# gnychis/gnuradio-3.5.0-dmr

Measured on AMD Instinct MI355X. Metric: Msamples/s through FIR->demod chain @256 taps, higher is better.
Workload: dtype f32 (FIR operands split into two binary16 halves on the matrix cores, f32 accumulation; demodulator f32)

## Files before the change

### gnuradio-3.5.0-dmr_amd/csrc/fir_mfma.hip

```cpp
#include <cstdio>
#include <cstdlib>

#include "device_math.h"
#include "fir_kernels.h"
#include "grhip_internal.h"
#include "mfma_tables.h"

#ifndef GRHIP_LG_W2
#define GRHIP_LG_W2 0
#endif
#ifndef GRHIP_LG_ACC3
#define GRHIP_LG_ACC3 0
#endif
#ifndef GRHIP_LG_ORDER
#define GRHIP_LG_ORDER 1
#endif
#ifndef GRHIP_MF_WGS
#define GRHIP_MF_WGS 2
#endif
#ifndef GRHIP_LG_SPF
#define GRHIP_LG_SPF 0
#endif
#ifndef GRHIP_LG_MAX4
#define GRHIP_LG_MAX4 0
#endif
#ifndef GRHIP_LG_EPI2
#define GRHIP_LG_EPI2 0
#endif
#ifndef GRHIP_LG_STAGE2
#define GRHIP_LG_STAGE2 1
#endif
#ifndef GRHIP_LG_LEAN
#define GRHIP_LG_LEAN 0
#endif
#ifndef GRHIP_LG_SPREAD
#define GRHIP_LG_SPREAD 0
#endif


namespace grhip {

typedef _Float16 h16x8 __attribute__((ext_vector_type(8)));
typedef _Float16 h16x2 __attribute__((ext_vector_type(2)));
typedef float f32x4 __attribute__((ext_vector_type(4)));
typedef float f32x2 __attribute__((ext_vector_type(2)));
typedef unsigned int u32x4 __attribute__((ext_vector_type(4)));
typedef unsigned int u32x2 __attribute__((ext_vector_type(2)));
typedef const float __attribute__((address_space(4))) *cfloat_cp;

namespace {

__host__ __device__ constexpr int ilog2c(int v) { return v <= 1 ? 0 : 1 + ilog2c(v >> 1); }

constexpr int SCR_SEG = 36;
constexpr int SCR_WAVE = mf::SEGS * SCR_SEG;

template <int D, int KS> struct Geo {
    static constexpr int Q = mf::SEG_OUT * D;
    static constexpr int LOGQ = ilog2c(Q);
    static constexpr int CB = mf::BLK * D / mf::CHUNK;
    static constexpr int NCH = mf::chunks_per_seg(D, KS);
    static constexpr int SP = mf::tile_samples(D, KS);
    static constexpr int NI = mf::rounds(D, KS);
    static constexpr int PL = mf::plane_bytes(D, KS);
    static constexpr int HALO = NCH * mf::CHUNK - (mf::SEGS * mf::SEG_OUT - mf::WAVE_NEW) * D - (mf::SEGS - 1) * 0;
    static constexpr int OFF_ATAN = 4 * PL;
    static constexpr int OFF_MISC = OFF_ATAN + 256 * 8;
    static constexpr int OFF_G = OFF_MISC + 32;
    static constexpr int LDS = OFF_G + mf::NG * 64 * 16;
    static_assert((1 << LOGQ) == Q, "segment stride must be a power of two");
    static_assert(HALO >= 0 && HALO % 32 == 0, "halo");
    static_assert(mf::NBLK != 4 || mf::plane_pos(mf::WAVE_NEW * D - 1, D) + 2 - mf::plane_pos(HALO, D) >= SCR_WAVE * 4, "a wave's own stretch of a plane must hold one accumulator tile");
    static_assert(mf::ROUND % Q == 0, "a staging round must cover whole segment strides");
};

#define GRHIP_DPPF(v, ctrl, rmask, bc) \
    __builtin_bit_cast(float, __builtin_amdgcn_update_dpp(0, __builtin_bit_cast(int, (v)), (ctrl), (rmask), 0xf, (bc)))
__device__ __forceinline__ float wave_max_nonneg(float x)
{
    x = __builtin_fmaxf(x, GRHIP_DPPF(x, 0xB1, 0xf, true));
    x = __builtin_fmaxf(x, GRHIP_DPPF(x, 0x4E, 0xf, true));
    x = __builtin_fmaxf(x, GRHIP_DPPF(x, 0x141, 0xf, true));
    x = __builtin_fmaxf(x, GRHIP_DPPF(x, 0x140, 0xf, true));
    x = __builtin_fmaxf(x, GRHIP_DPPF(x, 0x142, 0xa, false));
    x = __builtin_fmaxf(x, GRHIP_DPPF(x, 0x143, 0xc, false));
    return __builtin_bit_cast(float, __builtin_amdgcn_readlane(__builtin_bit_cast(int, x), 63));
}

__device__ __forceinline__ float wave_sum_f(float x)
{
    x += GRHIP_DPPF(x, 0xB1, 0xf, true);
    x += GRHIP_DPPF(x, 0x4E, 0xf, true);
    x += GRHIP_DPPF(x, 0x141, 0xf, true);
    x += GRHIP_DPPF(x, 0x140, 0xf, true);
    x += GRHIP_DPPF(x, 0x142, 0xa, false);
    x += GRHIP_DPPF(x, 0x143, 0xc, false);
    return __builtin_bit_cast(float, __builtin_amdgcn_readlane(__builtin_bit_cast(int, x), 63));
}

template <int CTRL>
__device__ __forceinline__ float dpp_row(float v)
{
    return __builtin_bit_cast(float, __builtin_amdgcn_update_dpp(0, __builtin_bit_cast(int, v), CTRL, 0xf, 0xf, true));
}

__device__ __forceinline__ h16x2 split_lo(f32x2 x, h16x2 hi)
{
    unsigned lo;
    const unsigned h = __builtin_bit_cast(unsigned, hi);
    asm("v_fma_mixlo_f16 %0, %1, 1.0, -%2 op_sel_hi:[0,0,1]" : "=v"(lo) : "v"(x.x), "v"(h));
    asm("v_fma_mixhi_f16 %0, %1, 1.0, -%2 op_sel:[0,0,1] op_sel_hi:[0,0,1]" : "+v"(lo) : "v"(x.y), "v"(h));
    return __builtin_bit_cast(h16x2, lo);
}

__device__ __forceinline__ void split_scaled(float x0, float x1, float s, h16x2 &hi, h16x2 &lo)
{
    unsigned h, l;
    asm("v_fma_mixlo_f16 %0, %1, %2, 0" : "=v"(h) : "v"(x0), "v"(s));
    asm("v_fma_mixhi_f16 %0, %1, %2, 0" : "+v"(h) : "v"(x1), "v"(s));
    asm("v_fma_mixlo_f16 %0, %1, %2, -%3 op_sel_hi:[0,0,1]" : "=v"(l) : "v"(x0), "v"(s), "v"(h));
    asm("v_fma_mixhi_f16 %0, %1, %2, -%3 op_sel:[0,0,1] op_sel_hi:[0,0,1]" : "+v"(l) : "v"(x1), "v"(s), "v"(h));
    hi = __builtin_bit_cast(h16x2, h);
    lo = __builtin_bit_cast(h16x2, l);
}

#ifdef GRHIP_STAMP
__device__ unsigned long long *g_mf_stamp_buf = nullptr;
__device__ __forceinline__ unsigned long long mf_stamp_now()
{
    unsigned long long t;
    __builtin_amdgcn_sched_barrier(0);
    asm volatile("s_memrealtime %0\n\ts_waitcnt lgkmcnt(0)" : "=s"(t) :: "memory");
    __builtin_amdgcn_sched_barrier(0);
    return t;
}
#define MF_STAMP_DECL unsigned long long st_acc[8] = {0, 0, 0, 0, 0, 0, 0, 0}, st_last = mf_stamp_now(), st_begin = st_last
#define MF_STAMP(k) do { unsigned long long n__ = mf_stamp_now(); st_acc[k] += n__ - st_last; st_last = n__; } while (0)
#define MF_STAMP_OUT(nwaves) do { if ((threadIdx.x & 63) == 0 && g_mf_stamp_buf) { \
        unsigned long long *o__ = g_mf_stamp_buf + ((size_t)blockIdx.x * (nwaves) + (threadIdx.x >> 6)) * 10; \
        for (int k__ = 0; k__ < 8; ++k__) o__[k__] = st_acc[k__]; \
        o__[8] = st_begin; o__[9] = mf_stamp_now(); } } while (0)
#else
#define MF_STAMP_DECL
#define MF_STAMP(k)
#define MF_STAMP_OUT(nwaves)
#endif

struct AtanPairs {
    const f32x2 *p;
    __device__ __forceinline__ f32x2 operator[](int k) const { return p[k]; }
};

}

template <int D, int KS, bool PREMIX, int EPI, bool TAPQ = false>
__global__ void __launch_bounds__(mf::THREADS, GRHIP_MF_WGS) fir_mfma_kernel(const FirMfmaArgs a)
{
    static_assert(!TAPQ || PREMIX, "the tap-angle correction belongs to freq_xlating's pre-mix form");
    using G = Geo<D, KS>;
    constexpr int NI = G::NI, PL = G::PL, LOGQ = G::LOGQ, CB = G::CB, SP = G::SP;
    constexpr bool DEMOD = EPI == EPI_DEMOD;
    constexpr bool ROT = EPI == EPI_ROTATE;
    static_assert(!DEMOD || PREMIX, "the fused demodulator belongs to the pre-mix form");
    static_assert(EPI == EPI_DEMOD || EPI == EPI_ROTATE || EPI == EPI_NONE, "epilogue");
    constexpr int NTE = mf::NTE, BLK = mf::BLK, NBLK = mf::NBLK;

    extern __shared__ __attribute__((aligned(256))) unsigned char smem[];
    const AtanPairs s_atan{reinterpret_cast<const f32x2 *>(smem + G::OFF_ATAN)};
    float *wmax = reinterpret_cast<float *>(smem + G::OFF_MISC);
    unsigned *sched_slot = reinterpret_cast<unsigned *>(smem + G::OFF_MISC + 16);

    const int t = threadIdx.x, lane = t & 63, w = t >> 6;
    const int tiles_per_stream = (int)((a.n_out + NTE - 1) / NTE);

    h16x8 Ah[KS], Al[KS];
    {
        const h16x8 *Ag = reinterpret_cast<const h16x8 *>(a.A);
#pragma unroll
        for (int js = 0; js < KS; ++js) {
            Ah[js] = Ag[(js * 2 + 0) * 64 + lane];
            Al[js] = Ag[(js * 2 + 1) * 64 + lane];
        }
    }
    constexpr int JG0 = mf::g_first(KS);
    if (TAPQ) {
        const h16x8 *Gg = reinterpret_cast<const h16x8 *>(a.A) + (size_t)KS * 2 * 64;
        if (t < mf::NG * 64) reinterpret_cast<h16x8 *>(smem + G::OFF_G)[t] = Gg[t];
    }
    const float tq_sgn = __builtin_amdgcn_ldexpf((lane & 8) ? 1.0f : -1.0f, -mf::G_EXTRA_EXP);
    f32x2 wl{1.f, 0.f}, wl1{1.f, 0.f};
    if (PREMIX) {
        const float2 v = a.wlane[t];
        wl = f32x2{v.x, v.y};
        wl1 = cmul_pk(wl, f32x2{a.wstep.x, a.wstep.y});
    }
    const cfloat_cp stab = (cfloat_cp)a.stab;
    if (DEMOD) {
        f32x2 *at = reinterpret_cast<f32x2 *>(smem + G::OFF_ATAN);
        for (int i = t; i < 256; i += mf::THREADS)
            at[i] = GRHIP_LG_LEAN ? f32x2{a.atan_tab[i], a.atan_tab[i + 1] - a.atan_tab[i]} : f32x2{a.atan_tab[i], a.atan_tab[i + 1]};
    }
    const int st_off = 4 * t + 32 * ((2 * t) >> LOGQ);
    constexpr int ST_STEP = 2 * mf::ROUND + 32 * (mf::ROUND >> LOGQ);
    const int col = lane & 15, part = col >> 3, sl = col & 7, g = lane >> 4;
    const int rd_u = w * (mf::WAVE_NEW * D) + (sl << LOGQ) + 8 * g;
    const int rd_plane = part * 2 * PL;
    const int scw_u = w * (mf::WAVE_NEW * D) + G::HALO;
    float *scw = reinterpret_cast<float *>(smem + 2 * scw_u + 32 * (scw_u >> LOGQ));
    const int sc_wr = sl * SCR_SEG + 8 * g + part;
    const int rsl = lane >> 3, r8 = lane & 7;
    const int sc_rd = rsl * SCR_SEG + 4 * r8;

    f32x4 pf[NI];

    const int lead = a.off ^ (int)(a.n_lo & 1);
    auto tile_geom = [&](int s, int b, __amdgpu_buffer_rsrc_t &rsrc, int &voff) __attribute__((always_inline)) {
        const long long g0 = ((long long)b * NTE - BLK) * D - a.off - a.n_lo + lead;
        const float2 *x = a.x + (long long)s * a.x_stride + a.n_lo - lead;
        const long long bytes = (a.n_in - a.n_lo + lead) * 8;
        rsrc = __builtin_amdgcn_make_buffer_rsrc(const_cast<float2 *>(x), 0, (int)bytes, 0x00020000);
        voff = (int)(g0 * 8) + 16 * t;
    };
    auto fetch = [&](__amdgpu_buffer_rsrc_t rsrc, int voff, int part_) __attribute__((always_inline)) {
        constexpr int PER = (NI + NBLK - 1) / NBLK;
#pragma unroll
        for (int i = 0; i < NI; ++i) {
            if (part_ >= 0 && i / PER != part_) continue;
            int vo = voff + i * (16 * mf::THREADS);
            if ((i + 1) * mf::ROUND > SP && 2 * t + i * mf::ROUND >= SP) vo = 0x7ffff000;
            const u32x4 v = __builtin_amdgcn_raw_buffer_load_b128(rsrc, vo, 0, 0);
            pf[i] = __builtin_bit_cast(f32x4, v);
        }
    };

    [[maybe_unused]] auto fetch_one = [&](__amdgpu_buffer_rsrc_t rsrc, int voff, int i) __attribute__((always_inline)) {
        int vo = voff + i * (16 * mf::THREADS);
        if ((i + 1) * mf::ROUND > SP && 2 * t + i * mf::ROUND >= SP) vo = 0x7ffff000;
        const u32x4 v = __builtin_amdgcn_raw_buffer_load_b128(rsrc, vo, 0, 0);
        pf[i] = __builtin_bit_cast(f32x4, v);
    };
    const unsigned total_tiles = (unsigned)tiles_per_stream * (unsigned)a.n_streams;
    const unsigned Gd = gridDim.x;
    unsigned cur = blockIdx.x, nxt = cur + Gd;
    auto decode = [&](unsigned id, int &s_, int &b_) __attribute__((always_inline)) {
        b_ = (int)(id / (unsigned)a.n_streams);
        s_ = (int)(id - (unsigned)b_ * (unsigned)a.n_streams);
    };
    int s = 0, bidx = 0;
    decode(cur, s, bidx);
    if (cur < total_tiles) {
        __amdgpu_buffer_rsrc_t rsrc; int voff;
        tile_geom(s, bidx, rsrc, voff);
        fetch(rsrc, voff, -1);
    }
    unsigned nn_q = 0;
    int voff_cur = 0;
    if (lead) {
        __amdgpu_buffer_rsrc_t rsrc;
        tile_geom(s, bidx, rsrc, voff_cur);
    }

    MF_STAMP_DECL;
    while (cur < total_tiles) {
        int s_nxt, b_nxt;
        MF_STAMP(7);

#if GRHIP_LG_STAGE2
        f32x2 Sa_first{0.f, 0.f}, Sb_first{0.f, 0.f};
        if (PREMIX && GRHIP_LG_SPF) { Sa_first = f32x2{stab[0], stab[1]}; Sb_first = f32x2{stab[2], stab[3]}; }
#endif
        {
            float m = 0.f, m1 = 0.f, m2 = 0.f, m3 = 0.f;
#pragma unroll
            for (int i = 0; i < NI; ++i) {
                if (GRHIP_LG_MAX4 && (i & 1)) {
                    asm("v_max3_f32 %0, |%1|, |%2|, %0" : "+v"(m2) : "v"(pf[i][0]), "v"(pf[i][1]));
                    asm("v_max3_f32 %0, |%1|, |%2|, %0" : "+v"(m3) : "v"(pf[i][2]), "v"(pf[i][3]));
                } else {
                    asm("v_max3_f32 %0, |%1|, |%2|, %0" : "+v"(m) : "v"(pf[i][0]), "v"(pf[i][1]));
                    asm("v_max3_f32 %0, |%1|, |%2|, %0" : "+v"(GRHIP_LG_MAX4 ? m1 : m) : "v"(pf[i][2]), "v"(pf[i][3]));
                }
            }
            if (GRHIP_LG_MAX4) {
                asm("v_max3_f32 %0, %1, %2, %0" : "+v"(m) : "v"(m1), "v"(m2));
                asm("v_max3_f32 %0, %1, %1, %0" : "+v"(m) : "v"(m3));
            }
            m = wave_max_nonneg(m);
            if (!(m < __builtin_inff())) {
                float mf = 0.f;
#pragma unroll
                for (int i = 0; i < NI; ++i)
#pragma unroll
                    for (int e = 0; e < 4; ++e) {
                        const float av = __builtin_fabsf(pf[i][e]);
                        mf = av < __builtin_inff() ? __builtin_fmaxf(mf, av) : mf;
                    }
                m = wave_max_nonneg(mf);
            }
            if (lane == 0) wmax[w] = m;
            if (a.sched && t == 0) sched_slot[0] = nn_q + 2u * Gd;
        }
        MF_STAMP(0);
        __syncthreads();
        MF_STAMP(1);
        if (a.sched && cur != blockIdx.x) nxt = sched_slot[0];
        nxt = (unsigned)__builtin_amdgcn_readfirstlane((int)nxt);
        decode(nxt, s_nxt, b_nxt);
        float scale, inv_scale;
        {
            const float mt = __builtin_fmaxf(__builtin_fmaxf(wmax[0], wmax[1]), __builtin_fmaxf(wmax[2], wmax[3]));
            int k = 14 - __builtin_amdgcn_frexp_expf(mt);
            k = k > 100 ? 100 : (k < -100 ? -100 : k);
            scale = __builtin_amdgcn_ldexpf(1.0f, k);
            inv_scale = __builtin_amdgcn_ldexpf(1.0f, -k - a.kexp);
        }

        if (lead && bidx == 0) {
#pragma unroll
            for (int i = 0; i < NI; ++i)
                if (voff_cur + i * (16 * mf::THREADS) == 0) { pf[i][0] = 0.f; pf[i][1] = 0.f; }
        }
#if defined(GRHIP_DIAG) && defined(GRHIP_MF_EXP)
        const bool exp_off = a.n_out < 0;
#define MF_EXP_SKIP(bit) if (!((GRHIP_MF_EXP & (bit)) && !exp_off))
#else
#define MF_EXP_SKIP(bit)
#endif
#if GRHIP_LG_STAGE2
        if (PREMIX) MF_EXP_SKIP(2)
        {
            const f32x2 ws0 = wl * scale, ws1 = wl1 * scale;
            unsigned char *dst = smem + st_off;
            auto store_round = [&](int i, unsigned rh, unsigned rlo, unsigned ih, unsigned ilo) __attribute__((always_inline)) {
                if ((i + 1) * mf::ROUND <= SP || 2 * t + i * mf::ROUND < SP) {
                    unsigned char *d = dst + i * ST_STEP;
                    *reinterpret_cast<unsigned *>(d) = rh;
                    *reinterpret_cast<unsigned *>(d + PL) = rlo;
                    *reinterpret_cast<unsigned *>(d + 2 * PL) = ih;
                    *reinterpret_cast<unsigned *>(d + 3 * PL) = ilo;
                }
            };
#define MF_CM1(t, a, b) "v_pk_mul_f32 " t ", " a ", " b " op_sel:[1,1] op_sel_hi:[1,0] neg_lo:[0,1]\n\t"
#define MF_CM2(r, a, b, t) "v_pk_fma_f32 " r ", " a ", " b ", " t " op_sel_hi:[0,1,1]\n\t"
            int i = 0;
            f32x2 Sa = Sa_first, Sb = Sb_first;
            if (!GRHIP_LG_SPF) { Sa = f32x2{stab[0], stab[1]}; Sb = f32x2{stab[2], stab[3]}; }
#pragma unroll
            for (; i + 1 < NI; i += 2) {
                f32x2 Sa_n = Sa, Sb_n = Sb;
                if (GRHIP_LG_SPF) {
                    if (i + 2 < NI) Sa_n = f32x2{stab[2 * i + 4], stab[2 * i + 5]};
                    if (i + 3 < NI) Sb_n = f32x2{stab[2 * i + 6], stab[2 * i + 7]};
                } else if (i > 0) {
                    Sa = f32x2{stab[2 * i], stab[2 * i + 1]}; Sb = f32x2{stab[2 * i + 2], stab[2 * i + 3]};
                }
                f32x2 a0{pf[i][0], pf[i][1]}, a1{pf[i][2], pf[i][3]}, b0{pf[i + 1][0], pf[i + 1][1]}, b1{pf[i + 1][2], pf[i + 1][3]};
                f32x2 t0, t1, t2, t3, p0, p1, p2, p3;
                unsigned arh, aih, arl, ail, brh, bih, brl, bil;
                asm(MF_CM1("%0", "%12", "%14") MF_CM1("%1", "%13", "%14") MF_CM1("%2", "%12", "%15") MF_CM1("%3", "%13", "%15")
                    MF_CM2("%4", "%12", "%14", "%0") MF_CM2("%5", "%13", "%14", "%1") MF_CM2("%6", "%12", "%15", "%2") MF_CM2("%7", "%13", "%15", "%3")
                    MF_CM1("%0", "%8", "%4") MF_CM1("%1", "%9", "%5") MF_CM1("%2", "%10", "%6") MF_CM1("%3", "%11", "%7")
                    MF_CM2("%8", "%8", "%4", "%0") MF_CM2("%9", "%9", "%5", "%1") MF_CM2("%10", "%10", "%6", "%2") "v_pk_fma_f32 %11, %11, %7, %3 op_sel_hi:[0,1,1]"
                    : "=&v"(t0), "=&v"(t1), "=&v"(t2), "=&v"(t3), "=&v"(p0), "=&v"(p1), "=&v"(p2), "=&v"(p3),
                      "+v"(a0), "+v"(a1), "+v"(b0), "+v"(b1)
                    : "v"(ws0), "v"(ws1), "s"(Sa), "s"(Sb));
                asm("v_cvt_pk_f16_f32 %0, %8, %10\n\t"
                    "v_cvt_pk_f16_f32 %1, %9, %11\n\t"
                    "v_cvt_pk_f16_f32 %4, %12, %14\n\t"
                    "v_cvt_pk_f16_f32 %5, %13, %15\n\t"
                    "v_fma_mixlo_f16 %2, %8, 1.0, -%0 op_sel_hi:[0,0,1]\n\t"
                    "v_fma_mixlo_f16 %3, %9, 1.0, -%1 op_sel_hi:[0,0,1]\n\t"
                    "v_fma_mixlo_f16 %6, %12, 1.0, -%4 op_sel_hi:[0,0,1]\n\t"
                    "v_fma_mixlo_f16 %7, %13, 1.0, -%5 op_sel_hi:[0,0,1]\n\t"
                    "v_fma_mixhi_f16 %2, %10, 1.0, -%0 op_sel:[0,0,1] op_sel_hi:[0,0,1]\n\t"
                    "v_fma_mixhi_f16 %3, %11, 1.0, -%1 op_sel:[0,0,1] op_sel_hi:[0,0,1]\n\t"
                    "v_fma_mixhi_f16 %6, %14, 1.0, -%4 op_sel:[0,0,1] op_sel_hi:[0,0,1]\n\t"
                    "v_fma_mixhi_f16 %7, %15, 1.0, -%5 op_sel:[0,0,1] op_sel_hi:[0,0,1]"
                    : "=&v"(arh), "=&v"(aih), "=&v"(arl), "=&v"(ail), "=&v"(brh), "=&v"(bih), "=&v"(brl), "=&v"(bil)
                    : "v"(a0.x), "v"(a0.y), "v"(a1.x), "v"(a1.y), "v"(b0.x), "v"(b0.y), "v"(b1.x), "v"(b1.y));
                store_round(i, arh, arl, aih, ail);
                store_round(i + 1, brh, brl, bih, bil);
                if (GRHIP_LG_SPF) { Sa = Sa_n; Sb = Sb_n; }
            }
            if (i < NI) {
                const f32x2 S = GRHIP_LG_SPF ? Sa : f32x2{stab[2 * i], stab[2 * i + 1]};
                f32x2 e0{pf[i][0], pf[i][1]}, e1{pf[i][2], pf[i][3]};
                e0 = cmul_pk(e0, cmul_pk(ws0, S));
                e1 = cmul_pk(e1, cmul_pk(ws1, S));
                const f32x2 re{e0.x, e1.x}, im{e0.y, e1.y};
                const h16x2 rh = __builtin_convertvector(re, h16x2), ih = __builtin_convertvector(im, h16x2);
                const h16x2 rlo = split_lo(re, rh), ilo = split_lo(im, ih);
                store_round(i, __builtin_bit_cast(unsigned, rh), __builtin_bit_cast(unsigned, rlo), __builtin_bit_cast(unsigned, ih),
                            __builtin_bit_cast(unsigned, ilo));
            }
#undef MF_CM1
#undef MF_CM2
        }
        else
#endif
        MF_EXP_SKIP(2)
        {
            const f32x2 ws0 = wl * scale, ws1 = wl1 * scale;
            unsigned char *dst = smem + st_off;
#pragma unroll
            for (int i = 0; i < NI; ++i) {
                f32x2 e0{pf[i][0], pf[i][1]}, e1{pf[i][2], pf[i][3]};
                if (PREMIX) {
#if defined(GRHIP_DIAG) && defined(GRHIP_PROBE) && (GRHIP_PROBE & 2)
                    const double ang0 = a.omega * (double)(2 * t + mf::ROUND * i - a.off);
                    const f32x2 p0{(float)cos(ang0) * scale, (float)sin(ang0) * scale};
                    const f32x2 p1{(float)cos(ang0 + a.omega) * scale, (float)sin(ang0 + a.omega) * scale};
                    e0 = cmul_pk(e0, p0);
                    e1 = cmul_pk(e1, p1);
#else
                    const f32x2 S{stab[2 * i], stab[2 * i + 1]};
                    e0 = cmul_pk(e0, cmul_pk(ws0, S));
                    e1 = cmul_pk(e1, cmul_pk(ws1, S));
#endif
                } else {
                    e0 = e0 * scale;
                    e1 = e1 * scale;
                }
                const f32x2 re{e0.x, e1.x}, im{e0.y, e1.y};
                const h16x2 rh = __builtin_convertvector(re, h16x2), ih = __builtin_convertvector(im, h16x2);
                const h16x2 rlo = split_lo(re, rh), ilo = split_lo(im, ih);
                if ((i + 1) * mf::ROUND <= SP || 2 * t + i * mf::ROUND < SP) {
#if GRHIP_LG_W2
                    const int ad = st_off + i * ST_STEP;
                    asm volatile("ds_write2st64_b32 %0, %1, %2 offset0:0 offset1:%5\n\t"
                                 "ds_write2st64_b32 %0, %3, %4 offset0:%6 offset1:%7"
                                 :: "v"(ad), "v"(rh), "v"(rlo), "v"(ih), "v"(ilo),
                                    "n"(PL / 256), "n"(2 * (PL / 256)), "n"(3 * (PL / 256)) : "memory");
#else
                    unsigned char *d = dst + i * ST_STEP;
                    *reinterpret_cast<h16x2 *>(d) = rh;
                    *reinterpret_cast<h16x2 *>(d + PL) = rlo;
                    *reinterpret_cast<h16x2 *>(d + 2 * PL) = ih;
                    *reinterpret_cast<h16x2 *>(d + 3 * PL) = ilo;
#endif
                }
            }
        }
        float2 ypf = make_float2(0.f, 0.f);
        if (DEMOD && bidx == 0 && a.y_prev) {
            const float2 yp = a.y_prev[s];
            const float2 vm = a.vtab[BLK - 1];
            const float2 q = cmul_fma(yp, make_float2(vm.x, -vm.y));
            const float sc2 = __builtin_amdgcn_ldexpf(scale, a.kexp);
            ypf = make_float2(q.x * sc2, q.y * sc2);
        }
        MF_STAMP(2);
        __syncthreads();
        MF_STAMP(3);

        __amdgpu_buffer_rsrc_t rsrc_n; int voff_n;
        tile_geom(s_nxt, b_nxt, rsrc_n, voff_n);
        if (nxt >= total_tiles) voff_n = 0x7ffff000 - NI * 16 * mf::THREADS;
        if (a.sched && t == 0) nn_q = atomicAdd(a.sched, 1u);

        constexpr int OOB = 0x7ffffff0;
        __amdgpu_buffer_rsrc_t orsrc, grsrc;
        if (DEMOD) {
            orsrc = __builtin_amdgcn_make_buffer_rsrc(a.d_out + (long long)s * a.d_stride, 0, (int)(a.n_out * 4), 0x00020000);
        } else {
            orsrc = __builtin_amdgcn_make_buffer_rsrc(a.y_out + (long long)s * a.y_stride, 0, (int)(a.n_out * 8), 0x00020000);
            if (ROT) grsrc = __builtin_amdgcn_make_buffer_rsrc(const_cast<float2 *>(a.gtab), 0, (int)(a.n_out * 8), 0x00020000);
        }
        const int jt = w * mf::WAVE_NEW + rsl * mf::SEG_OUT + 2 * r8;
        const int n_base = bidx * NTE - BLK + jt;
        const bool first_of_stream = bidx == 0 && t == 7;
        float ypendx = 0.f, ypendy = 0.f;
        float d1_pend = 0.f;
        float y1x = 0.f, y1y = 0.f;
        const float ypfx = ypf.x, ypfy = ypf.y;

        auto epilogue = [&](int b, const f32x4 &v) __attribute__((always_inline)) {
            const float y0x = v[0], y0y = v[1];
            const float y1px = y1x, y1py = y1y;
            y1x = v[2]; y1y = v[3];
            const float2 y0 = make_float2(y0x, y0y);
            const int n = n_base + BLK * b;
            const bool own = !(b == 0 && rsl == 0) && n >= 0;
            if (DEMOD) {
                if (b == 0) {
                    y1x = first_of_stream ? ypfx : y1x;
                    y1y = first_of_stream ? ypfy : y1y;
                }
                float px = dpp_row<0x111>(y1x), py = dpp_row<0x111>(y1y);
                if (b > 0) {
                    const float cx = dpp_row<0x107>(y1px), cy = dpp_row<0x107>(y1py);
                    px = r8 == 0 ? cx : px;
                    py = r8 == 0 ? cy : py;
                } else {
                    ypendx = y0x; ypendy = y0y;
                }
                const float2 prev = make_float2(px, py), y1 = make_float2(y1x, y1y);
                const float d0 = GRHIP_LG_LEAN ? quad_demod_lean(y0, prev, a.gain, s_atan) : quad_demod_fast(y0, prev, a.gain, s_atan);
                const float d1 = GRHIP_LG_LEAN ? quad_demod_lean(y1, y0, a.gain, s_atan) : quad_demod_fast(y1, y0, a.gain, s_atan);
                if (b == 0) d1_pend = d1;
                const bool st_ok = own && !(b == 0 && r8 == 0);
                const f32x2 dd{d0, d1};
                __builtin_amdgcn_raw_buffer_store_b64(__builtin_bit_cast(u32x2, dd), orsrc, st_ok ? 4 * n : OOB, 0, 0);
            } else {
                float2 o0 = y0, o1 = make_float2(y1x, y1y);
                if (PREMIX) {
                    const float4 vv = *reinterpret_cast<const float4 *>(a.vtab + jt + BLK * b);
                    o0 = cmul_fma(o0, make_float2(vv.x, vv.y));
                    o1 = cmul_fma(o1, make_float2(vv.z, vv.w));
                }
                o0.x *= inv_scale; o0.y *= inv_scale; o1.x *= inv_scale; o1.y *= inv_scale;
                if (ROT) {
                    const u32x4 gv = __builtin_amdgcn_raw_buffer_load_b128(grsrc, own ? 8 * n : OOB, 0, 0);
                    const f32x4 gq = __builtin_bit_cast(f32x4, gv);
                    o0 = cmul_ref(o0, make_float2(gq[0], gq[1]));
                    o1 = cmul_ref(o1, make_float2(gq[2], gq[3]));
                }
                const f32x2 oa{o0.x, o0.y}, ob{o1.x, o1.y};
                const int so = own ? 8 * n : OOB;
                __builtin_amdgcn_raw_buffer_store_b64(__builtin_bit_cast(u32x2, oa), orsrc, so, 0, 0);
                __builtin_amdgcn_raw_buffer_store_b64(__builtin_bit_cast(u32x2, ob), orsrc, so + 8, 0, 0);
            }
        };

        auto chunk_ptr = [&](int c) __attribute__((always_inline)) {
            const int u = rd_u + mf::CHUNK * c;
            return smem + rd_plane + 2 * u + 32 * (u >> LOGQ);
        };
        f32x4 acc[NBLK];
#if defined(GRHIP_DIAG) && defined(GRHIP_MF_EXP) && (GRHIP_MF_EXP & 1)
#pragma unroll
        for (int b = 0; b < NBLK; ++b) acc[b] = f32x4{0.f, 0.f, 0.f, 0.f};
#pragma unroll
        for (int q = 0; q < 4; ++q) fetch(rsrc_n, voff_n, q);
        if (exp_off)
#endif
        {
        h16x8 Bh_n = *reinterpret_cast<const h16x8 *>(chunk_ptr(0));
        h16x8 Bl_n = *reinterpret_cast<const h16x8 *>(chunk_ptr(0) + PL);
#pragma unroll
        for (int b = 0; b < NBLK; ++b) {
#if GRHIP_LG_ACC3
            f32x4 m0{0.f, 0.f, 0.f, 0.f}, m1{0.f, 0.f, 0.f, 0.f}, lo{0.f, 0.f, 0.f, 0.f};
#else
            acc[b] = f32x4{0.f, 0.f, 0.f, 0.f};
#endif
            f32x4 tq{0.f, 0.f, 0.f, 0.f};
            auto kstep = [](int q) constexpr { return GRHIP_LG_ORDER ? ((q & 1) ? KS - 1 - (q >> 1) : (q >> 1)) : q; };
            h16x8 Gcur{}, Gnext{};
#pragma unroll
            for (int jq = 0; jq < KS; ++jq) {
                const int j = kstep(jq);
                const h16x8 Bh = Bh_n, Bl = Bl_n;
                if (TAPQ) {
                    Gcur = Gnext;
                    const int jn = jq + 1 < KS ? kstep(jq + 1) : (b + 1 < NBLK ? kstep(0) : -1);
                    if (jn >= JG0 && jn < JG0 + mf::NG) {
                        unsigned goff = (unsigned)(G::OFF_G + 16 * lane + (jn - JG0) * 1024);
                        asm volatile("" : "+v"(goff));
                        Gnext = *reinterpret_cast<const __attribute__((address_space(3))) h16x8 *>(goff);
                    }
                }
                const int cn = jq + 1 < KS ? CB * b + kstep(jq + 1) : CB * (b + 1) + kstep(0);
                if (jq + 1 < KS || b + 1 < NBLK) {
                    const unsigned char *src = chunk_ptr(cn);
                    Bh_n = *reinterpret_cast<const h16x8 *>(src);
                    Bl_n = *reinterpret_cast<const h16x8 *>(src + PL);
                }
#if GRHIP_LG_ACC3
                constexpr bool EVEN_ODD = GRHIP_LG_ACC3 == 1 && (KS <= 6 || (D == 4 && EPI == EPI_DEMOD));
                if (EVEN_ODD && (j & 1)) m1 = __builtin_amdgcn_mfma_f32_16x16x32_f16(Ah[j], Bh, m1, 0, 0, 0);
                else m0 = __builtin_amdgcn_mfma_f32_16x16x32_f16(Ah[j], Bh, m0, 0, 0, 0);
                lo = __builtin_amdgcn_mfma_f32_16x16x32_f16(Ah[j], Bl, lo, 0, 0, 0);
                lo = __builtin_amdgcn_mfma_f32_16x16x32_f16(Al[j], Bh, lo, 0, 0, 0);
#else
                acc[b] = __builtin_amdgcn_mfma_f32_16x16x32_f16(Ah[j], Bh, acc[b], 0, 0, 0);
                acc[b] = __builtin_amdgcn_mfma_f32_16x16x32_f16(Ah[j], Bl, acc[b], 0, 0, 0);
                acc[b] = __builtin_amdgcn_mfma_f32_16x16x32_f16(Al[j], Bh, acc[b], 0, 0, 0);
#endif
                if (TAPQ && j >= JG0 && j < JG0 + mf::NG) {
                    const u32x4 bw = __builtin_bit_cast(u32x4, Bh);
                    u32x4 sw;
#pragma unroll
                    for (int e = 0; e < 4; ++e)
                        sw[e] = (unsigned)__builtin_amdgcn_update_dpp((int)bw[e], (int)bw[e], 0x128, 0xf, 0xf, false);
                    tq = __builtin_amdgcn_mfma_f32_16x16x32_f16(Gcur, __builtin_bit_cast(h16x8, sw), tq, 0, 0, 0);
                }
#if GRHIP_LG_SPREAD
                {
                    constexpr int STEP = (NBLK * KS) / NI > 0 ? (NBLK * KS) / NI : 1;
                    const int pos = b * KS + jq;
                    if (pos % STEP == 0 && pos / STEP < NI) fetch_one(rsrc_n, voff_n, pos / STEP);
                }
#else
                if (jq == 1) fetch(rsrc_n, voff_n, b);
#endif
            }
#if GRHIP_LG_ACC3
            acc[b] = GRHIP_LG_ACC3 == 1 ? (m0 + m1) + lo : m0 + lo;
#endif
            if (TAPQ) {
#pragma unroll
                for (int e = 0; e < 4; ++e) acc[b][e] = __builtin_fmaf(tq_sgn, tq[e], acc[b][e]);
            }
        }
        }
        MF_STAMP(4);
        MF_EXP_SKIP(5)
        {
        __builtin_amdgcn_sched_barrier(0);
#pragma unroll
        for (int b = 0; b < NBLK; ++b) {
            float *sb = reinterpret_cast<float *>(reinterpret_cast<unsigned char *>(scw) + b * PL);
#pragma unroll
            for (int i = 0; i < 4; ++i) sb[sc_wr + 2 * i] = acc[b][i];
        }
        __builtin_amdgcn_fence(__ATOMIC_SEQ_CST, "wavefront");
        auto read_block = [&](int b) __attribute__((always_inline)) {
            return *reinterpret_cast<const f32x4 *>(reinterpret_cast<const unsigned char *>(scw) + b * PL + 4 * sc_rd);
        };
        f32x4 yv_n = read_block(0);
#pragma unroll
        for (int b = 0; b < NBLK; ++b) {
            const f32x4 yv = yv_n;
            if (b + 1 < NBLK) yv_n = read_block(b + 1);
            epilogue(b, yv);
            if (!GRHIP_LG_EPI2 || (b & 1) || !DEMOD) __builtin_amdgcn_sched_barrier(0);
        }
        if (DEMOD) {
            const float px = __shfl_up(y1x, 1), py = __shfl_up(y1y, 1);
            const float dp = GRHIP_LG_LEAN ? quad_demod_lean(make_float2(ypendx, ypendy), make_float2(px, py), a.gain, s_atan)
                                           : quad_demod_fast(make_float2(ypendx, ypendy), make_float2(px, py), a.gain, s_atan);
            const bool st_ok = r8 == 0 && rsl != 0 && n_base >= 0;
            const f32x2 dd{dp, d1_pend};
            __builtin_amdgcn_raw_buffer_store_b64(__builtin_bit_cast(u32x2, dd), orsrc, st_ok ? 4 * n_base : OOB, 0, 0);
            if (a.y_last && bidx == tiles_per_stream - 1 && w == 0) {
                const long long item0 = (a.n_out - 1) * D - a.n_lo + lead;
                __amdgpu_buffer_rsrc_t xr; int vdummy;
                tile_geom(s, bidx, xr, vdummy);
                float sx = 0.f, sy = 0.f;
                for (int i = lane; i < a.T; i += 64) {
                    const long long it = item0 + i;
                    const int vo = (it < 0 || (lead && it == 0)) ? OOB : (int)(it * 8);
                    const u32x2 xv = __builtin_amdgcn_raw_buffer_load_b64(xr, vo, 0, 0);
                    const f32x2 xf = __builtin_bit_cast(f32x2, xv);
                    const float2 c = a.ctaps[i];
                    sx = __builtin_fmaf(c.x, xf.x, sx); sx = __builtin_fmaf(-c.y, xf.y, sx);
                    sy = __builtin_fmaf(c.x, xf.y, sy); sy = __builtin_fmaf(c.y, xf.x, sy);
                }
                sx = wave_sum_f(sx); sy = wave_sum_f(sy);
                if (lane == 0) a.y_last[s] = make_float2(sx, sy);
            }
        }

        }
        MF_STAMP(5);
        cur = nxt;
        if (!a.sched) nxt = nxt + Gd;
        s = s_nxt; bidx = b_nxt;
        voff_cur = voff_n;
    }
    if (a.sched && t == 0) {
        __threadfence();
        if (atomicAdd(a.sched + 1, 1u) == Gd - 1) {
            a.sched[0] = 0;
            a.sched[1] = 0;
            __threadfence();
        }
    }
#ifdef GRHIP_STAMP
    if (lane == 0 && g_mf_stamp_buf) {
        unsigned long long *o = g_mf_stamp_buf + ((size_t)blockIdx.x * mf::WAVES + w) * 10;
        for (int k = 0; k < 8; ++k) o[k] = st_acc[k];
        o[8] = st_begin; o[9] = mf_stamp_now();
    }
#endif
}

#ifdef GRHIP_STAMP
extern "C" __attribute__((visibility("default"))) int grdbg_set_stamp_buffer_mfma(void *d_buf)
{
    unsigned long long *p = (unsigned long long *)d_buf;
    GRHIP_HIP(hipMemcpyToSymbol(HIP_SYMBOL(g_mf_stamp_buf), &p, sizeof(p)));
    return GRHIP_OK;
}
#endif


#if defined(GRHIP_DIAG) && GRHIP_MF_NBLK == 4
#ifndef GRHIP_RS_ABL
#define GRHIP_RS_ABL 0
#endif
namespace rs {
constexpr int NSTG = 8, NMAT = mf::WAVES;
constexpr int THREADS = 64 * (NSTG + NMAT);
constexpr int STG_T = 64 * NSTG;
constexpr int ROUND = 2 * STG_T;
#ifndef GRHIP_RS_PD
#define GRHIP_RS_PD 2
#endif
constexpr int PD = GRHIP_RS_PD;
static_assert(mf::NBLK == 4 && NSTG == 2 * NMAT, "two stagers share a matrix wave's four blocks");
}

namespace {
template <int D, int KS> struct GeoRS {
    using G = Geo<D, KS>;
    static constexpr int NI = (G::SP + rs::ROUND - 1) / rs::ROUND;
    static constexpr int BUF = 4 * G::PL;
    static constexpr int OFF_ATAN = 2 * BUF;
    static constexpr int OFF_MISC = OFF_ATAN + 256 * 8;
    static constexpr int LDS = OFF_MISC + 64;
    static_assert(rs::ROUND % G::Q == 0, "a staging round must cover whole segment strides");
    static_assert(2 * (NI - 1) < G::NI, "the stagers' round phasors are every other entry of the 512-sample table");
    static_assert(LDS <= 160 * 1024, "LDS");
};

__device__ __forceinline__ void rs_barrier()
{
    asm volatile("s_waitcnt lgkmcnt(0)\n\ts_barrier" ::: "memory");
}
}

template <int D, int KS, bool PREMIX, int EPI>
__global__ void __launch_bounds__(rs::THREADS, 1) fir_mfma_rs_kernel(const FirMfmaArgs a)
{
    using G = Geo<D, KS>;
    using R = GeoRS<D, KS>;
    constexpr int NI = R::NI, PL = G::PL, LOGQ = G::LOGQ, CB = G::CB, SP = G::SP;
    constexpr bool DEMOD = EPI == EPI_DEMOD;
    constexpr bool ROT = EPI == EPI_ROTATE;
    static_assert(!DEMOD || PREMIX, "the fused demodulator belongs to the pre-mix form");
    constexpr int NTE = mf::NTE, BLK = mf::BLK, NBLK = mf::NBLK;

    extern __shared__ __attribute__((aligned(256))) unsigned char smem[];
    const AtanPairs s_atan{reinterpret_cast<const f32x2 *>(smem + R::OFF_ATAN)};
    float *wmax = reinterpret_cast<float *>(smem + R::OFF_MISC);

    const int t = threadIdx.x, lane = t & 63;
    const int w = __builtin_amdgcn_readfirstlane(t >> 6);
    const int tiles_per_stream = (int)((a.n_out + NTE - 1) / NTE);
    const unsigned total_tiles = (unsigned)tiles_per_stream * (unsigned)a.n_streams;
    const unsigned Gd = gridDim.x;
    const int n_my = (int)((total_tiles - blockIdx.x + Gd - 1) / Gd);
    const int P = n_my + 3;

    const int ts = t;
    constexpr int OOB = 0x7ffffff0;
    const int lead = a.off ^ (int)(a.n_lo & 1);
    int *kring = reinterpret_cast<int *>(smem + R::OFF_MISC + 32);
    auto decode = [&](int q, int &s_, int &b_) __attribute__((always_inline)) {
        const unsigned id = blockIdx.x + (unsigned)q * Gd;
        b_ = (int)(id / (unsigned)a.n_streams);
        s_ = (int)(id - (unsigned)b_ * (unsigned)a.n_streams);
    };
    auto tile_geom = [&](int s, int b, __amdgpu_buffer_rsrc_t &rsrc, int &voff) __attribute__((always_inline)) {
        const long long g0 = ((long long)b * NTE - BLK) * D - a.off - a.n_lo + lead;
        const float2 *x = a.x + (long long)s * a.x_stride + a.n_lo - lead;
        const long long bytes = (a.n_in - a.n_lo + lead) * 8;
        rsrc = __builtin_amdgcn_make_buffer_rsrc(const_cast<float2 *>(x), 0, (int)bytes, 0x00020000);
        voff = (int)(g0 * 8) + 16 * ts;
    };
    const int rsl = lane >> 3, r8 = lane & 7;
    struct EpiRegs { f32x4 yv; f32x2 pv; };
    auto epilogue_read = [&](int q, int mw, int b, EpiRegs &er) __attribute__((always_inline)) {
        const int scw_u = mw * (mf::WAVE_NEW * D) + G::HALO;
        const unsigned char *scr = smem + (q & 1) * R::BUF + 2 * scw_u + 32 * (scw_u >> LOGQ);
        er.yv = *reinterpret_cast<const f32x4 *>(scr + b * PL + 4 * (rsl * SCR_SEG + 4 * r8));
        er.pv = f32x2{0.f, 0.f};
        if (DEMOD) {
            const int pb = b == 0 ? NBLK - 1 : b - 1;
            const int ps = b == 0 ? (rsl > 0 ? rsl - 1 : 0) : rsl;
            er.pv = *reinterpret_cast<const f32x2 *>(scr + pb * PL + 4 * (ps * SCR_SEG + 30));
        }
    };
    auto epilogue_block = [&](int q, int kx, int mw, int b, bool carry_out, const EpiRegs &er) __attribute__((always_inline)) {
        int s, bidx;
        decode(q, s, bidx);
        const float inv_scale = __builtin_amdgcn_ldexpf(1.0f, -kx - a.kexp);
        float ypfx = 0.f, ypfy = 0.f;
        if (DEMOD && bidx == 0 && b == 1 && a.y_prev) {
            const float2 yp = a.y_prev[s];
            const float2 vm = a.vtab[BLK - 1];
            const float2 qq = cmul_fma(yp, make_float2(vm.x, -vm.y));
            const float sc2 = __builtin_amdgcn_ldexpf(1.0f, kx + a.kexp);
            ypfx = qq.x * sc2; ypfy = qq.y * sc2;
        }
        __amdgpu_buffer_rsrc_t orsrc, grsrc;
        if (DEMOD) {
            orsrc = __builtin_amdgcn_make_buffer_rsrc(a.d_out + (long long)s * a.d_stride, 0, (int)(a.n_out * 4), 0x00020000);
        } else {
            orsrc = __builtin_amdgcn_make_buffer_rsrc(a.y_out + (long long)s * a.y_stride, 0, (int)(a.n_out * 8), 0x00020000);
            if (ROT) grsrc = __builtin_amdgcn_make_buffer_rsrc(const_cast<float2 *>(a.gtab), 0, (int)(a.n_out * 8), 0x00020000);
        }
        const int jt = mw * mf::WAVE_NEW + rsl * mf::SEG_OUT + 2 * r8;
        const int n_base = bidx * NTE - BLK + jt;
        {
            const float y0x = er.yv[0], y0y = er.yv[1], y1x = er.yv[2], y1y = er.yv[3];
            const int n = n_base + BLK * b;
            const bool own = !(b == 0 && rsl == 0) && n >= 0;
            if (DEMOD) {
                float px = dpp_row<0x111>(y1x), py = dpp_row<0x111>(y1y);
                const bool from_carry = bidx == 0 && mw == 0 && b == 1 && rsl == 0;
                const float qx = from_carry ? ypfx : er.pv[0], qy = from_carry ? ypfy : er.pv[1];
                px = r8 == 0 ? qx : px;
                py = r8 == 0 ? qy : py;
                const float d0 = quad_demod_fast(make_float2(y0x, y0y), make_float2(px, py), a.gain, s_atan);
                const float d1 = quad_demod_fast(make_float2(y1x, y1y), make_float2(y0x, y0y), a.gain, s_atan);
                const f32x2 dd{d0, d1};
                __builtin_amdgcn_raw_buffer_store_b64(__builtin_bit_cast(u32x2, dd), orsrc, own ? 4 * n : OOB, 0, 0);
            } else {
                float2 o0 = make_float2(y0x, y0y), o1 = make_float2(y1x, y1y);
                if (PREMIX) {
                    const float4 vv = *reinterpret_cast<const float4 *>(a.vtab + jt + BLK * b);
                    o0 = cmul_fma(o0, make_float2(vv.x, vv.y));
                    o1 = cmul_fma(o1, make_float2(vv.z, vv.w));
                }
                o0.x *= inv_scale; o0.y *= inv_scale; o1.x *= inv_scale; o1.y *= inv_scale;
                if (ROT) {
                    const u32x4 gv = __builtin_amdgcn_raw_buffer_load_b128(grsrc, own ? 8 * n : OOB, 0, 0);
                    const f32x4 gq = __builtin_bit_cast(f32x4, gv);
                    o0 = cmul_ref(o0, make_float2(gq[0], gq[1]));
                    o1 = cmul_ref(o1, make_float2(gq[2], gq[3]));
                }
                const f32x2 oa{o0.x, o0.y}, ob{o1.x, o1.y};
                const int so = own ? 8 * n : OOB;
                __builtin_amdgcn_raw_buffer_store_b64(__builtin_bit_cast(u32x2, oa), orsrc, so, 0, 0);
                __builtin_amdgcn_raw_buffer_store_b64(__builtin_bit_cast(u32x2, ob), orsrc, so + 8, 0, 0);
            }
        }
        if (carry_out && DEMOD && a.y_last && bidx == tiles_per_stream - 1) {
            const long long item0 = (a.n_out - 1) * D - a.n_lo + lead;
            __amdgpu_buffer_rsrc_t xr; int vdummy;
            tile_geom(s, bidx, xr, vdummy);
            float sx = 0.f, sy = 0.f;
            for (int i = lane; i < a.T; i += 64) {
                const long long it = item0 + i;
                const int vo = (it < 0 || (lead && it == 0)) ? OOB : (int)(it * 8);
                const u32x2 xv = __builtin_amdgcn_raw_buffer_load_b64(xr, vo, 0, 0);
                const f32x2 xf = __builtin_bit_cast(f32x2, xv);
                const float2 c = a.ctaps[i];
                sx = __builtin_fmaf(c.x, xf.x, sx); sx = __builtin_fmaf(-c.y, xf.y, sx);
                sy = __builtin_fmaf(c.x, xf.y, sy); sy = __builtin_fmaf(c.y, xf.x, sy);
            }
            sx = wave_sum_f(sx); sy = wave_sum_f(sy);
            if (lane == 0) a.y_last[s] = make_float2(sx, sy);
        }
    };

    if (w >= rs::NSTG) {
        const int mw = w - rs::NSTG;
#if defined(GRHIP_RS_PRIO) && GRHIP_RS_PRIO == 2
        __builtin_amdgcn_s_setprio(1);
#endif
        h16x8 Ah[KS], Al[KS];
        {
            const h16x8 *Ag = reinterpret_cast<const h16x8 *>(a.A);
#pragma unroll
            for (int js = 0; js < KS; ++js) {
                Ah[js] = Ag[(js * 2 + 0) * 64 + lane];
                Al[js] = Ag[(js * 2 + 1) * 64 + lane];
            }
        }
        const int col = lane & 15, part = col >> 3, sl = col & 7, g = lane >> 4;
        const int wu = mw * (mf::WAVE_NEW * D);
        const int rd_lane = part * 2 * PL + 2 * ((sl << LOGQ) + 8 * g) + 32 * sl;
        auto chunk_off = [&](int c) __attribute__((always_inline)) {
            const int u = wu + mf::CHUNK * c;
            return 2 * u + 32 * (u >> LOGQ);
        };
        const int scw_u = wu + G::HALO;
        const int scw_off = 2 * scw_u + 32 * (scw_u >> LOGQ);
        const int sc_wr = sl * SCR_SEG + 8 * g + part;

        MF_STAMP_DECL;
        constexpr int NCH = G::NCH;
        constexpr int PDK = KS > 6 ? 1 : rs::PD;
        for (int p = 0; p < P; ++p) {
            const bool act = p >= 2 && p - 2 < n_my;
            unsigned char *buf = smem + (p & 1) * R::BUF;
            f32x4 m0[NBLK], m1[NBLK], lo[NBLK];
            h16x8 Bh[PDK + 1], Bl[PDK + 1];
            auto ld = [&](int c) __attribute__((always_inline)) {
                const unsigned char *src = buf + rd_lane + chunk_off(c);
                Bh[c % (PDK + 1)] = *reinterpret_cast<const h16x8 *>(src);
                Bl[c % (PDK + 1)] = *reinterpret_cast<const h16x8 *>(src + PL);
            };
            auto half = [&](int h) __attribute__((always_inline)) {
                constexpr int HC = NCH / 8;
                if (h == 0) {
#pragma unroll
                    for (int b = 0; b < NBLK; ++b) {
                        m0[b] = f32x4{0.f, 0.f, 0.f, 0.f};
                        m1[b] = f32x4{0.f, 0.f, 0.f, 0.f};
                        lo[b] = f32x4{0.f, 0.f, 0.f, 0.f};
                    }
#pragma unroll
                    for (int c = 0; c < PDK; ++c) ld(c);
                }
#pragma unroll
                for (int c = h * HC; c < (h ? NCH : HC); ++c) {
                    if (c + PDK < NCH) ld(c + PDK);
                    __builtin_amdgcn_sched_barrier(0);
                    const int sl_ = c % (PDK + 1);
#pragma unroll
                    for (int b = 0; b < NBLK; ++b) {
                        const int j = c - CB * b;
                        if (j < 0 || j >= KS) continue;
                        if (j & 1) m1[b] = __builtin_amdgcn_mfma_f32_16x16x32_f16(Ah[j], Bh[sl_], m1[b], 0, 0, 0);
                        else m0[b] = __builtin_amdgcn_mfma_f32_16x16x32_f16(Ah[j], Bh[sl_], m0[b], 0, 0, 0);
                    }
#pragma unroll
                    for (int b = 0; b < NBLK; ++b) {
                        const int j = c - CB * b;
                        if (j < 0 || j >= KS) continue;
                        lo[b] = __builtin_amdgcn_mfma_f32_16x16x32_f16(Ah[j], Bl[sl_], lo[b], 0, 0, 0);
                    }
#pragma unroll
                    for (int b = 0; b < NBLK; ++b) {
                        const int j = c - CB * b;
                        if (j < 0 || j >= KS) continue;
                        lo[b] = __builtin_amdgcn_mfma_f32_16x16x32_f16(Al[j], Bh[sl_], lo[b], 0, 0, 0);
                    }
                    __builtin_amdgcn_sched_barrier(0);
                }
            };
            MF_STAMP(7);
            if (act && !(GRHIP_RS_ABL & 1)) half(0);
            MF_STAMP(0);
            rs_barrier();
            MF_STAMP(3);
            if (act) {
                if (!(GRHIP_RS_ABL & 1)) half(1);
                else {
#pragma unroll
                    for (int b = 0; b < NBLK; ++b) { m0[b] = f32x4{0.f, 0.f, 0.f, 0.f}; m1[b] = m0[b]; lo[b] = m0[b]; }
                }
#pragma unroll
                for (int b = 0; b < NBLK; ++b) {
                    const f32x4 accf = (m0[b] + m1[b]) + lo[b];
                    float *sb = reinterpret_cast<float *>(buf + scw_off + b * PL);
#pragma unroll
                    for (int i = 0; i < 4; ++i) sb[sc_wr + 2 * i] = accf[i];
                }
                const int q = p - 2;
                const int kx = kring[q & 3];
#pragma unroll
                for (int b = 2; b < NBLK; ++b) {
                    if (GRHIP_RS_ABL & 2) break;
                    EpiRegs er;
                    epilogue_read(q, mw, b, er);
                    epilogue_block(q, kx, mw, b, false, er);
                }
            }
            MF_STAMP(4);
            rs_barrier();
            MF_STAMP(5);
// ... 256 lines not shown
```

Baseline: 534,400.

## Run demod epilogue straight from MFMA accumulator layout via cross-lane permutes

The epilogue used to write each wave's accumulator blocks to an LDS scratch area and read them back transposed so each lane held consecutive output samples. It now consumes the accumulators in their native MFMA lane layout. A row DPP swap pairs real and imaginary parts, and ds_bpermute fetches the previous sample for the differential demodulator. This removes the scratch writes, the wave fence and the reloads, at the cost of extra permute instructions and remapped store indices. An optional flag (EPIX, off by default) also interleaves each block's epilogue into the MFMA loop.

```diff
diff --git a/gnuradio-3.5.0-dmr_amd/csrc/fir_mfma.hip b/gnuradio-3.5.0-dmr_amd/csrc/fir_mfma.hip
--- a/gnuradio-3.5.0-dmr_amd/csrc/fir_mfma.hip
+++ b/gnuradio-3.5.0-dmr_amd/csrc/fir_mfma.hip
@@ -24,8 +24,11 @@
 #ifndef GRHIP_LG_MAX4
 #define GRHIP_LG_MAX4 0
 #endif
-#ifndef GRHIP_LG_EPI2
-#define GRHIP_LG_EPI2 0
+#ifndef GRHIP_LG_EPIX
+#define GRHIP_LG_EPIX 0
+#endif
+#ifndef GRHIP_LG_EPIAT
+#define GRHIP_LG_EPIAT 0
 #endif
 #ifndef GRHIP_LG_STAGE2
 #define GRHIP_LG_STAGE2 1
@@ -164,6 +167,7 @@
     static_assert(!DEMOD || PREMIX, "the fused demodulator belongs to the pre-mix form");
     static_assert(EPI == EPI_DEMOD || EPI == EPI_ROTATE || EPI == EPI_NONE, "epilogue");
     constexpr int NTE = mf::NTE, BLK = mf::BLK, NBLK = mf::NBLK;
+    constexpr bool EPI_X = DEMOD && GRHIP_LG_EPIX;
 
     extern __shared__ __attribute__((aligned(256))) unsigned char smem[];
     const AtanPairs s_atan{reinterpret_cast<const f32x2 *>(smem + G::OFF_ATAN)};
@@ -205,11 +209,9 @@
     const int col = lane & 15, part = col >> 3, sl = col & 7, g = lane >> 4;
     const int rd_u = w * (mf::WAVE_NEW * D) + (sl << LOGQ) + 8 * g;
     const int rd_plane = part * 2 * PL;
-    const int scw_u = w * (mf::WAVE_NEW * D) + G::HALO;
-    float *scw = reinterpret_cast<float *>(smem + 2 * scw_u + 32 * (scw_u >> LOGQ));
-    const int sc_wr = sl * SCR_SEG + 8 * g + part;
-    const int rsl = lane >> 3, r8 = lane & 7;
-    const int sc_rd = rsl * SCR_SEG + 4 * r8;
+    const bool pt1 = part != 0;
+    const bool head = lane < 8;
+    const int bp_prev = ((lane - 8) & 63) << 2;
 
     f32x4 pf[NI];
 
@@ -323,8 +325,10 @@
 #if defined(GRHIP_DIAG) && defined(GRHIP_MF_EXP)
         const bool exp_off = a.n_out < 0;
 #define MF_EXP_SKIP(bit) if (!((GRHIP_MF_EXP & (bit)) && !exp_off))
+        const bool EPI_ON = !((GRHIP_MF_EXP & 5) && !exp_off);
 #else
 #define MF_EXP_SKIP(bit)
+        constexpr bool EPI_ON = true;
 #endif
 #if GRHIP_LG_STAGE2
         if (PREMIX) MF_EXP_SKIP(2)
@@ -466,39 +470,42 @@
             orsrc = __builtin_amdgcn_make_buffer_rsrc(a.y_out + (long long)s * a.y_stride, 0, (int)(a.n_out * 8), 0x00020000);
             if (ROT) grsrc = __builtin_amdgcn_make_buffer_rsrc(const_cast<float2 *>(a.gtab), 0, (int)(a.n_out * 8), 0x00020000);
         }
-        const int jt = w * mf::WAVE_NEW + rsl * mf::SEG_OUT + 2 * r8;
+        const int jt = w * mf::WAVE_NEW + sl * mf::SEG_OUT + 4 * g + 2 * part;
         const int n_base = bidx * NTE - BLK + jt;
-        const bool first_of_stream = bidx == 0 && t == 7;
+        const bool first_of_stream = bidx == 0 && t == 56;
         float ypendx = 0.f, ypendy = 0.f;
         float d1_pend = 0.f;
-        float y1x = 0.f, y1y = 0.f;
+        float cx = 0.f, cy = 0.f;
         const float ypfx = ypf.x, ypfy = ypf.y;
 
         auto epilogue = [&](int b, const f32x4 &v) __attribute__((always_inline)) {
-            const float y0x = v[0], y0y = v[1];
-            const float y1px = y1x, y1py = y1y;
-            y1x = v[2]; y1y = v[3];
+            const float s0 = pt1 ? v[0] : v[2], s1 = pt1 ? v[1] : v[3];
+            const float r0 = dpp_row<0x128>(s0), r1 = dpp_row<0x128>(s1);
+            const float y0x = pt1 ? r0 : v[0], y0y = pt1 ? v[2] : r0;
+            float y1x = pt1 ? r1 : v[1], y1y = pt1 ? v[3] : r1;
             const float2 y0 = make_float2(y0x, y0y);
             const int n = n_base + BLK * b;
-            const bool own = !(b == 0 && rsl == 0) && n >= 0;
+            const bool own = !(b == 0 && sl == 0) && n >= 0;
             if (DEMOD) {
                 if (b == 0) {
                     y1x = first_of_stream ? ypfx : y1x;
                     y1y = first_of_stream ? ypfy : y1y;
                 }
-                float px = dpp_row<0x111>(y1x), py = dpp_row<0x111>(y1y);
+                const float qx = __builtin_bit_cast(float, __builtin_amdgcn_ds_bpermute(bp_prev, __builtin_bit_cast(int, y1x)));
+                const float qy = __builtin_bit_cast(float, __builtin_amdgcn_ds_bpermute(bp_prev, __builtin_bit_cast(int, y1y)));
+                float px = qx, py = qy;
                 if (b > 0) {
-                    const float cx = dpp_row<0x107>(y1px), cy = dpp_row<0x107>(y1py);
-                    px = r8 == 0 ? cx : px;
-                    py = r8 == 0 ? cy : py;
+                    px = head ? cx : px;
+                    py = head ? cy : py;
                 } else {
                     ypendx = y0x; ypendy = y0y;
                 }
+                cx = qx; cy = qy;
                 const float2 prev = make_float2(px, py), y1 = make_float2(y1x, y1y);
                 const float d0 = GRHIP_LG_LEAN ? quad_demod_lean(y0, prev, a.gain, s_atan) : quad_demod_fast(y0, prev, a.gain, s_atan);
                 const float d1 = GRHIP_LG_LEAN ? quad_demod_lean(y1, y0, a.gain, s_atan) : quad_demod_fast(y1, y0, a.gain, s_atan);
                 if (b == 0) d1_pend = d1;
-                const bool st_ok = own && !(b == 0 && r8 == 0);
+                const bool st_ok = own && !(b == 0 && head);
                 const f32x2 dd{d0, d1};
                 __builtin_amdgcn_raw_buffer_store_b64(__builtin_bit_cast(u32x2, dd), orsrc, st_ok ? 4 * n : OOB, 0, 0);
             } else {
@@ -594,6 +601,7 @@
 #else
                 if (jq == 1) fetch(rsrc_n, voff_n, b);
 #endif
+                if (EPI_X && EPI_ON && b > 0 && jq == GRHIP_LG_EPIAT) epilogue(b - 1, acc[b - 1]);
             }
 #if GRHIP_LG_ACC3
             acc[b] = GRHIP_LG_ACC3 == 1 ? (m0 + m1) + lo : m0 + lo;
@@ -605,53 +613,41 @@
         }
         }
         MF_STAMP(4);
-        MF_EXP_SKIP(5)
-        {
-        __builtin_amdgcn_sched_barrier(0);
-#pragma unroll
-        for (int b = 0; b < NBLK; ++b) {
-            float *sb = reinterpret_cast<float *>(reinterpret_cast<unsigned char *>(scw) + b * PL);
-#pragma unroll
-            for (int i = 0; i < 4; ++i) sb[sc_wr + 2 * i] = acc[b][i];
-        }
-        __builtin_amdgcn_fence(__ATOMIC_SEQ_CST, "wavefront");
-        auto read_block = [&](int b) __attribute__((always_inline)) {
-            return *reinterpret_cast<const f32x4 *>(reinterpret_cast<const unsigned char *>(scw) + b * PL + 4 * sc_rd);
-        };
-        f32x4 yv_n = read_block(0);
-#pragma unroll
-        for (int b = 0; b < NBLK; ++b) {
-            const f32x4 yv = yv_n;
-            if (b + 1 < NBLK) yv_n = read_block(b + 1);
-            epilogue(b, yv);
-            if (!GRHIP_LG_EPI2 || (b & 1) || !DEMOD) __builtin_amdgcn_sched_barrier(0);
-        }
-        if (DEMOD) {
-            const float px = __shfl_up(y1x, 1), py = __shfl_up(y1y, 1);
-            const float dp = GRHIP_LG_LEAN ? quad_demod_lean(make_float2(ypendx, ypendy), make_float2(px, py), a.gain, s_atan)
-                                           : quad_demod_fast(make_float2(ypendx, ypendy), make_float2(px, py), a.gain, s_atan);
-            const bool st_ok = r8 == 0 && rsl != 0 && n_base >= 0;
-            const f32x2 dd{dp, d1_pend};
-            __builtin_amdgcn_raw_buffer_store_b64(__builtin_bit_cast(u32x2, dd), orsrc, st_ok ? 4 * n_base : OOB, 0, 0);
-            if (a.y_last && bidx == tiles_per_stream - 1 && w == 0) {
-                const long long item0 = (a.n_out - 1) * D - a.n_lo + lead;
-                __amdgpu_buffer_rsrc_t xr; int vdummy;
-                tile_geom(s, bidx, xr, vdummy);
-                float sx = 0.f, sy = 0.f;
-                for (int i = lane; i < a.T; i += 64) {
-                    const long long it = item0 + i;
-                    const int vo = (it < 0 || (lead && it == 0)) ? OOB : (int)(it * 8);
-                    const u32x2 xv = __builtin_amdgcn_raw_buffer_load_b64(xr, vo, 0, 0);
-                    const f32x2 xf = __builtin_bit_cast(f32x2, xv);
-                    const float2 c = a.ctaps[i];
-                    sx = __builtin_fmaf(c.x, xf.x, sx); sx = __builtin_fmaf(-c.y, xf.y, sx);
-                    sy = __builtin_fmaf(c.x, xf.y, sy); sy = __builtin_fmaf(c.y, xf.x, sy);
-                }
-                sx = wave_sum_f(sx); sy = wave_sum_f(sy);
-                if (lane == 0) a.y_last[s] = make_float2(sx, sy);
-            }
-        }
-
+        if (EPI_ON) {
+            if (!EPI_X) {
+                __builtin_amdgcn_sched_barrier(0);
+#pragma unroll
+                for (int b = 0; b + 1 < NBLK; ++b) {
+                    epilogue(b, acc[b]);
+                    __builtin_amdgcn_sched_barrier(0);
+                }
+            }
+            epilogue(NBLK - 1, acc[NBLK - 1]);
+            if (DEMOD) {
+                const float px = dpp_row<0x111>(cx), py = dpp_row<0x111>(cy);
+                const float dp = GRHIP_LG_LEAN ? quad_demod_lean(make_float2(ypendx, ypendy), make_float2(px, py), a.gain, s_atan)
+                                               : quad_demod_fast(make_float2(ypendx, ypendy), make_float2(px, py), a.gain, s_atan);
+                const bool st_ok = head && sl != 0 && n_base >= 0;
+                const f32x2 dd{dp, d1_pend};
+                __builtin_amdgcn_raw_buffer_store_b64(__builtin_bit_cast(u32x2, dd), orsrc, st_ok ? 4 * n_base : OOB, 0, 0);
+                if (a.y_last && bidx == tiles_per_stream - 1 && w == 0) {
+                    const long long item0 = (a.n_out - 1) * D - a.n_lo + lead;
+                    __amdgpu_buffer_rsrc_t xr; int vdummy;
+                    tile_geom(s, bidx, xr, vdummy);
+                    float sx = 0.f, sy = 0.f;
+                    for (int i = lane; i < a.T; i += 64) {
+                        const long long it = item0 + i;
+                        const int vo = (it < 0 || (lead && it == 0)) ? OOB : (int)(it * 8);
+                        const u32x2 xv = __builtin_amdgcn_raw_buffer_load_b64(xr, vo, 0, 0);
+                        const f32x2 xf = __builtin_bit_cast(f32x2, xv);
+                        const float2 c = a.ctaps[i];
+                        sx = __builtin_fmaf(c.x, xf.x, sx); sx = __builtin_fmaf(-c.y, xf.y, sx);
+                        sy = __builtin_fmaf(c.x, xf.y, sy); sy = __builtin_fmaf(c.y, xf.x, sy);
+                    }
+                    sx = wave_sum_f(sx); sy = wave_sum_f(sy);
+                    if (lane == 0) a.y_last[s] = make_float2(sx, sy);
+                }
+            }
         }
         MF_STAMP(5);
         cur = nxt;
```

After: 534,500 (median of 6 runs). About the same (+0.0%).
